# eth-cscs/conflux

Hardware: NVIDIA H100
Metric: LU GFLOP/s (FP64, (2/3)N^3) (higher is better)
Workload: dtype f64

## Files before the change

### conflux_b200/csrc/panel.cu

```cuda
#include <cooperative_groups.h>

#include <climits>
#include <cstdlib>

#include "common.cuh"
#include "kernels.h"

namespace cflx {

namespace {
constexpr int PT_THREADS = 256;
constexpr int PT_WARPS = PT_THREADS / 32;
constexpr int PT_LAUNCH = PT_THREADS + 32;
constexpr int PT_ALLWARPS = PT_LAUNCH / 32;
constexpr int MAXG = 132;
constexpr int RPT_LIMIT = 8;

struct PanelArgs {
    double* W;
    int64_t ldw;
    int n, v, nsteps;
    int R, Rpad, G;
    int* perm_out;
    double* A00;
    uint2* slot_hdr;
    uint2* slot_rows;
    int epoch_base;
};

__device__ __forceinline__ void st_ll(uint2* p, unsigned data, unsigned epoch) {
    asm volatile("st.volatile.global.v2.u32 [%0], {%1, %2};" ::"l"(p), "r"(data), "r"(epoch) : "memory");
}
__device__ __forceinline__ uint4 ld_ll2(const uint2* p) {
    uint4 v;
    asm volatile("ld.volatile.global.v4.u32 {%0, %1, %2, %3}, [%4];" : "=r"(v.x), "=r"(v.y), "=r"(v.z), "=r"(v.w) : "l"(p) : "memory");
    return v;
}

struct Cand {
    unsigned long long key;
    int pos;
    int row;
};

__device__ __forceinline__ Cand warp_argmax(Cand c) {
    const unsigned hi = (unsigned)(c.key >> 32), lo = (unsigned)c.key;
    const unsigned m1 = __reduce_max_sync(0xffffffffu, hi);
    bool in = (hi == m1);
    const unsigned m2 = __reduce_max_sync(0xffffffffu, in ? lo : 0u);
    in = in && (lo == m2);
    const unsigned m3 = __reduce_min_sync(0xffffffffu, in ? (unsigned)c.pos : (unsigned)INT_MAX);
    const unsigned ballot = __ballot_sync(0xffffffffu, in && (unsigned)c.pos == m3);
    const int src = __ffs(ballot) - 1;
    Cand r;
    r.key = ((unsigned long long)m1 << 32) | m2;
    r.pos = (int)m3;
    r.row = __shfl_sync(0xffffffffu, c.row, src);
    return r;
}
__device__ __forceinline__ bool better(const Cand& a, const Cand& b) {
    return a.key > b.key || (a.key == b.key && a.pos < b.pos);
}
__device__ __forceinline__ Cand block_argmax(Cand c, unsigned long long* red_key, int* red_pos, int* red_row, int& rb) {
    Cand w = warp_argmax(c);
    const int warp = threadIdx.x >> 5, lane = threadIdx.x & 31;
    const int o = rb * PT_ALLWARPS;
    rb ^= 1;
    if (lane == 0) {
        red_key[o + warp] = w.key;
        red_pos[o + warp] = w.pos;
        red_row[o + warp] = w.row;
    }
    __syncthreads();
    Cand x{0ull, INT_MAX, -1};
    if (lane < PT_ALLWARPS) x = Cand{red_key[o + lane], red_pos[o + lane], red_row[o + lane]};
    return warp_argmax(x);
}

template <int NB, int RPT_MAX>
__global__ void __launch_bounds__(PT_LAUNCH, 1) panel_getrf_kernel(PanelArgs p) {
    extern __shared__ __align__(16) unsigned char smem_raw[];
    double* Ab = reinterpret_cast<double*>(smem_raw);
    double* U12 = Ab + (size_t)NB * p.Rpad;
    double* LU11 = U12 + (size_t)NB * p.v;
    double* prow = LU11 + NB * (NB + 1);
    unsigned long long* red_key = reinterpret_cast<unsigned long long*>(prow + 2 * (NB + 1));
    int* red_pos = reinterpret_cast<int*>(red_key + 2 * PT_ALLWARPS);
    int* red_row = red_pos + 2 * PT_ALLWARPS;
    int* pivrow_blk = red_row + 2 * PT_ALLWARPS;
    int* win_sh = pivrow_blk + NB;
    unsigned char* s_act = reinterpret_cast<unsigned char*>(win_sh + 4);
    int rb = 0;

    const int t = threadIdx.x, warp = t >> 5, lane = t & 31;
    const bool owner = t < PT_THREADS;
    const bool small = p.G <= 32;
    const bool fetcher = warp == (small ? PT_WARPS : 0);
    const int cta = blockIdx.x;
    const int row_base = cta * p.R;
    const int Rloc = max(0, min(p.R, p.n - row_base));
    const int Rpad = p.Rpad, v = p.v;
    double* __restrict__ W = p.W;
    const int64_t ldw = p.ldw;

    int pos[RPT_MAX];
    bool active[RPT_MAX];
#pragma unroll
    for (int q = 0; q < RPT_MAX; ++q) {
        const int lr = t + q * PT_THREADS;
        pos[q] = row_base + lr;
        active[q] = owner && lr < Rloc;
    }
    for (int lr = t; lr < Rpad; lr += PT_LAUNCH) s_act[lr] = lr < Rloc ? 1 : 0;

    for (int jb = 0; jb < p.nsteps; jb += NB) {
        const int nbc = min(NB, v - jb);
        const int nsb = min(nbc, p.nsteps - jb);
        for (int e = t; e < nbc * Rpad; e += PT_LAUNCH) {
            const int c = e / Rpad, lr = e - c * Rpad;
            if (lr < Rloc) Ab[e] = W[(int64_t)(jb + c) * ldw + row_base + lr];
        }
        __syncthreads();

        auto local_candidate = [&](int col) -> Cand {
            Cand c{0ull, INT_MAX, -1};
#pragma unroll
            for (int q = 0; q < RPT_MAX; ++q) {
                const int lr = t + q * PT_THREADS;
                if (active[q]) {
                    Cand o{(unsigned long long)__double_as_longlong(fabs(Ab[col * Rpad + lr])), pos[q], row_base + lr};
                    if (better(o, c)) c = o;
                }
            }
            return block_argmax(c, red_key, red_pos, red_row, rb);
        };
        auto publish = [&](const Cand& mine, int jg, int jprev, const double* pw) {
            const unsigned epoch = (unsigned)(p.epoch_base + jg + 1);
            const int par = jg & 1;
            uint2* myhdr = p.slot_hdr + (size_t)(par * MAXG + cta) * 4;
            if (t < 4) {
                const unsigned w = t == 0 ? (unsigned)mine.key : t == 1 ? (unsigned)(mine.key >> 32)
                                 : t == 2 ? (unsigned)mine.pos : (unsigned)mine.row;
                st_ll(myhdr + t, w, epoch);
            }
            if (t < nbc) {
                double x = 0.0;
                if (mine.row >= 0) {
                    const int lrw = mine.row - row_base;
                    x = Ab[t * Rpad + lrw];
                    if (jprev >= 0 && t > jprev + 1) x = fma(-Ab[jprev * Rpad + lrw], pw[t], x);
                }
                const unsigned long long xb = (unsigned long long)__double_as_longlong(x);
                uint2* myrow = p.slot_rows + (size_t)(par * MAXG + cta) * 64 + 2 * t;
                st_ll(myrow, (unsigned)xb, epoch);
                st_ll(myrow + 1, (unsigned)(xb >> 32), epoch);
            }
        };
        {
            const Cand mine0 = local_candidate(0);
            if (t < 32) __threadfence();
            publish(mine0, jb, -1, nullptr);
        }
        for (int j = 0; j < nsb; ++j) {
            const int jg = jb + j;
            const int par = jg & 1;
            double* pr = prow + par * (NB + 1);
            if (!small || fetcher) {
                const unsigned epoch = (unsigned)(p.epoch_base + jg + 1);
                Cand gc{0ull, INT_MAX, -1};
                for (int g = small ? lane : t; g < p.G; g += small ? 32 : PT_LAUNCH) {
                    const uint2* h = p.slot_hdr + (size_t)(par * MAXG + g) * 4;
                    uint4 a, b;
                    do {
                        a = ld_ll2(h);
                        b = ld_ll2(h + 2);
                    } while (a.y != epoch || a.w != epoch || b.y != epoch || b.w != epoch);
                    Cand o{((unsigned long long)a.z << 32) | a.x, (int)b.x, (int)b.z};
                    if (better(o, gc)) gc = o;
                }
                const Cand w = small ? warp_argmax(gc) : block_argmax(gc, red_key, red_pos, red_row, rb);
                const int wslot = small ? __ffs(__ballot_sync(0xffffffffu, gc.row == w.row)) - 1 : w.row / p.R;
                if (fetcher && lane < nbc) {
                    const uint2* wr = p.slot_rows + (size_t)(par * MAXG + wslot) * 64 + 2 * lane;
                    uint4 a;
                    do {
                        a = ld_ll2(wr);
                    } while (a.y != epoch || a.w != epoch);
                    const double x = __longlong_as_double((long long)(((unsigned long long)a.z << 32) | a.x));
                    pr[lane] = x;
                    LU11[j * (NB + 1) + lane] = x;
                    if (lane == j) pr[NB] = x != 0.0 ? 1.0 / x : 0.0;
                }
                if (fetcher && lane == 0) {
                    win_sh[2 * par] = w.pos;
                    win_sh[2 * par + 1] = w.row;
                }
            }
            __syncthreads();
            Cand win;
            win.key = 0;
            win.pos = win_sh[2 * par];
            win.row = win_sh[2 * par + 1];
            if (t == 0) {
                pivrow_blk[j] = win.row;
                if (cta == 0) p.perm_out[jg] = win.row;
            }
            const double pivot = pr[j];
            const double rinv = pr[NB];
            const bool have_next = (j + 1 < nbc);
            const double pnext = have_next ? pr[j + 1] : 0.0;
            double lq[RPT_MAX];
#pragma unroll
            for (int q = 0; q < RPT_MAX; ++q) {
                const int lr = t + q * PT_THREADS;
                lq[q] = 0.0;
                if (!active[q]) continue;
                if (row_base + lr == win.row) {
                    active[q] = false;
                    s_act[lr] = 0;
                    continue;
                }
                if (pos[q] == jg) pos[q] = win.pos;
                if (pivot != 0.0) {
                    lq[q] = Ab[j * Rpad + lr] * rinv;
                    Ab[j * Rpad + lr] = lq[q];
                }
                if (have_next) Ab[(j + 1) * Rpad + lr] = fma(-lq[q], pnext, Ab[(j + 1) * Rpad + lr]);
            }
            if (j + 1 < nsb) {
                const Cand mine = local_candidate(j + 1);
                publish(mine, jg + 1, j, pr);
                __syncthreads();
            }
            if (owner) {
                double* __restrict__ ab = Ab;
#pragma unroll 4
                for (int c2 = j + 2; c2 < nbc; ++c2) {
                    const double pc = pr[c2];
#pragma unroll
                    for (int q = 0; q < RPT_MAX; ++q) {
                        const int lr = t + q * PT_THREADS;
                        if (active[q]) ab[c2 * Rpad + lr] = fma(-lq[q], pc, ab[c2 * Rpad + lr]);
                    }
                }
            }
        }

        __syncthreads();
        for (int e = t; e < nbc * Rpad; e += PT_LAUNCH) {
            const int c = e / Rpad, lr = e - c * Rpad;
            if (lr < Rloc) W[(int64_t)(jb + c) * ldw + row_base + lr] = Ab[e];
        }
        if (cta == 0 && p.A00 != nullptr) {
            for (int e = t; e < nsb * nbc; e += PT_LAUNCH) {
                const int i = e / nbc, c = e % nbc;
                p.A00[(size_t)(jb + i) * v + jb + c] = LU11[i * (NB + 1) + c];
            }
        }

        const int cstart = jb + nbc;
        const int rem = v - cstart;
        if (rem > 0) {
            __syncthreads();
            __threadfence();
            for (int cc = t; cc < rem; cc += PT_LAUNCH) {
                const double* col = W + (int64_t)(cstart + cc) * ldw;
                double u[NB];
#pragma unroll
                for (int i = 0; i < NB; ++i) u[i] = (i < nsb) ? ld_cg_f64(col + pivrow_blk[i]) : 0.0;
#pragma unroll
                for (int i = 1; i < NB; ++i) {
                    if (i < nsb) {
#pragma unroll
                        for (int s2 = 0; s2 < i; ++s2) u[i] -= LU11[i * (NB + 1) + s2] * u[s2];
                    }
                }
#pragma unroll
                for (int i = 0; i < NB; ++i) U12[i * v + cc] = u[i];
                if (cta == 0 && p.A00 != nullptr) {
#pragma unroll
                    for (int i = 0; i < NB; ++i)
                        if (i < nsb) p.A00[(size_t)(jb + i) * v + cstart + cc] = u[i];
                }
            }
            __syncthreads();
            auto update_row = [&](int lr, int cfirst, int cstep, bool tail) {
                double l[NB];
#pragma unroll
                for (int i = 0; i < NB; ++i) l[i] = (i < nsb) ? Ab[i * Rpad + lr] : 0.0;
                double* wp = W + (int64_t)cstart * ldw + row_base + lr;
                int cc = cfirst;
                double w0 = 0, w1 = 0, w2 = 0, w3 = 0;
                if (cc + 3 < rem) {
                    w0 = wp[(int64_t)cc * ldw];
                    w1 = wp[(int64_t)(cc + 1) * ldw];
                    w2 = wp[(int64_t)(cc + 2) * ldw];
                    w3 = wp[(int64_t)(cc + 3) * ldw];
                }
                for (; cc + 3 < rem; cc += cstep) {
                    double n0 = 0, n1 = 0, n2 = 0, n3 = 0;
                    const int cn = cc + cstep;
                    if (cn + 3 < rem) {
                        n0 = wp[(int64_t)cn * ldw];
                        n1 = wp[(int64_t)(cn + 1) * ldw];
                        n2 = wp[(int64_t)(cn + 2) * ldw];
                        n3 = wp[(int64_t)(cn + 3) * ldw];
                    }
#pragma unroll
                    for (int i = 0; i < NB; ++i) {
                        const double2 ua = *reinterpret_cast<const double2*>(U12 + i * v + cc);
                        const double2 ub = *reinterpret_cast<const double2*>(U12 + i * v + cc + 2);
                        w0 -= l[i] * ua.x;
                        w1 -= l[i] * ua.y;
                        w2 -= l[i] * ub.x;
                        w3 -= l[i] * ub.y;
                    }
                    wp[(int64_t)cc * ldw] = w0;
                    wp[(int64_t)(cc + 1) * ldw] = w1;
                    wp[(int64_t)(cc + 2) * ldw] = w2;
                    wp[(int64_t)(cc + 3) * ldw] = w3;
                    w0 = n0;
                    w1 = n1;
                    w2 = n2;
                    w3 = n3;
                }
                if (tail) {
                    for (int ct = rem & ~3; ct < rem; ++ct) {
                        double x = wp[(int64_t)ct * ldw];
#pragma unroll
                        for (int i = 0; i < NB; ++i) x -= l[i] * U12[i * v + ct];
                        wp[(int64_t)ct * ldw] = x;
                    }
                }
            };
            if (RPT_MAX == 1 && p.R < PT_THREADS) {
                const int nshare = PT_THREADS / p.R;
                const int lr = t % p.R, part = t / p.R;
                if (owner && part < nshare && lr < Rloc && s_act[lr]) update_row(lr, 4 * part, 4 * nshare, part == 0);
            } else {
#pragma unroll 1
                for (int q = 0; q < RPT_MAX; ++q) {
                    const int lr = t + q * PT_THREADS;
                    if (lr >= Rloc || !active[q]) continue;
                    update_row(lr, 0, 4, true);
                }
            }
        }
        __threadfence();
        __syncthreads();
    }
    if (cta == 0)
        for (int i = p.nsteps + t; i < v; i += PT_LAUNCH) p.perm_out[i] = i;
}

constexpr int SK_CB = 16;
struct StackArgs {
    double* W;
    int64_t ldw;
    int n, v;
    int* perm_out;
    int* ppos;
    unsigned* flags;
    unsigned* ticket;
    unsigned ticket_base, epoch;
};
__device__ __forceinline__ unsigned ld_acquire_u32(const unsigned* p) {
    unsigned v;
    asm volatile("ld.acquire.gpu.global.u32 %0, [%1];" : "=r"(v) : "l"(p) : "memory");
    return v;
}
__device__ __forceinline__ void st_release_u32(unsigned* p, unsigned v) {
    asm volatile("st.release.gpu.global.u32 [%0], %1;" ::"l"(p), "r"(v) : "memory");
}
__device__ __forceinline__ void cp_async16(double* smem_dst, const double* gsrc) {
    asm volatile("cp.async.cg.shared.global [%0], [%1], 16;" ::"r"(smem_u32(smem_dst)), "l"(gsrc) : "memory");
}
__device__ __forceinline__ void cp_async_commit() { asm volatile("cp.async.commit_group;" ::: "memory"); }
__device__ __forceinline__ void cp_async_wait_all() { asm volatile("cp.async.wait_all;" ::: "memory"); }

template <int NT>
__global__ void __launch_bounds__(NT, 1) stack_getrf_kernel(StackArgs p) {
    __shared__ double A12s[SK_CB][SK_CB + 1];
    __shared__ double L11s[SK_CB][SK_CB + 1];
    __shared__ double prow[2][SK_CB];
    __shared__ unsigned long long red_key[2][32];
    __shared__ int red_pos[2][32], red_row[2][32];
    __shared__ int pivs[SK_CB], ppos_s[SK_CB];
    __shared__ int s_cta;
    extern __shared__ __align__(16) double Ls[];
    const int t = threadIdx.x, warp = t >> 5, lane = t & 31, nw = blockDim.x >> 5;
    if (t == 0) s_cta = (int)(atomicAdd(p.ticket, 1u) - p.ticket_base);
    __syncthreads();
    const int c = s_cta, c0 = c * SK_CB;
    const bool valid = t < p.n;
    double* __restrict__ W = p.W;
    const int64_t ldw = p.ldw;
    double a[SK_CB];
#pragma unroll
    for (int j = 0; j < SK_CB; ++j) a[j] = valid ? W[(int64_t)(c0 + j) * ldw + t] : 0.0;
    int pos = t;
    int mypiv = -1;

    for (int b = 0; b < c; ++b) {
        if (t == 0)
            while (ld_acquire_u32(p.flags + b) != p.epoch) {}
        __syncthreads();
        if (t < SK_CB) {
            pivs[t] = ld_cg_s32(p.perm_out + b * SK_CB + t);
            ppos_s[t] = ld_cg_s32(p.ppos + b * SK_CB + t);
        }
        {
            const int half = blockDim.x >> 1, q = t % half, h = t / half;
            if (2 * q < p.n) {
                const double* lp = W + (int64_t)(b * SK_CB + 8 * h) * ldw + 2 * q;
#pragma unroll
                for (int k = 0; k < SK_CB / 2; ++k) cp_async16(Ls + (8 * h + k) * NT + 2 * q, lp + (int64_t)k * ldw);
            }
        }
        cp_async_commit();
        __syncthreads();
        int kk = -1;
        if (mypiv < 0) {
#pragma unroll
            for (int k = 0; k < SK_CB; ++k) {
                if (pivs[k] == t) kk = k;
                else if (kk < 0 && pos == b * SK_CB + k) pos = ppos_s[k];
            }
        }
        if (kk >= 0) {
#pragma unroll
            for (int j = 0; j < SK_CB; ++j) A12s[kk][j] = a[j];
#pragma unroll
            for (int k = 0; k < SK_CB; ++k) L11s[kk][k] = ld_cg_f64(W + (int64_t)(b * SK_CB + k) * ldw + t);
        }
        __syncthreads();
        if (t < SK_CB) {
#pragma unroll
            for (int i = 1; i < SK_CB; ++i) {
                double x = A12s[i][t];
#pragma unroll
                for (int s2 = 0; s2 < i; ++s2) x = fma(-L11s[i][s2], A12s[s2][t], x);
                A12s[i][t] = x;
            }
        }
        cp_async_wait_all();
        __syncthreads();
        if (kk >= 0) {
#pragma unroll
            for (int j = 0; j < SK_CB; ++j) a[j] = A12s[kk][j];
            mypiv = b * SK_CB + kk;
        } else if (mypiv < 0 && valid) {
#pragma unroll
            for (int k = 0; k < SK_CB; ++k) {
                const double lk = Ls[k * NT + t];
#pragma unroll
                for (int j = 0; j < SK_CB; ++j) a[j] = fma(-lk, A12s[k][j], a[j]);
            }
        }
    }

#pragma unroll
    for (int j = 0; j < SK_CB; ++j) {
        const int jg = c0 + j, par = j & 1;
        Cand cd{0ull, INT_MAX, -1};
        if (valid && mypiv < 0) cd = Cand{(unsigned long long)__double_as_longlong(fabs(a[j])), pos, t};
        const Cand w1 = warp_argmax(cd);
        if (lane == 0) {
            red_key[par][warp] = w1.key;
            red_pos[par][warp] = w1.pos;
            red_row[par][warp] = w1.row;
        }
        __syncthreads();
        Cand x{0ull, INT_MAX, -1};
        if (lane < nw) x = Cand{red_key[par][lane], red_pos[par][lane], red_row[par][lane]};
        const Cand win = warp_argmax(x);
        if (t == win.row) {
#pragma unroll
            for (int m = 0; m < SK_CB; ++m) prow[par][m] = a[m];
            mypiv = jg;
        }
        if (t == 0) {
            p.perm_out[jg] = win.row;
            p.ppos[jg] = win.pos;
        }
        __syncthreads();
        if (valid && mypiv < 0) {
            if (pos == jg) pos = win.pos;
            const double pivot = prow[par][j];
            const double rinv = pivot != 0.0 ? 1.0 / pivot : 0.0;
            double lq = 0.0;
            if (pivot != 0.0) {
                lq = a[j] * rinv;
                a[j] = lq;
            }
#pragma unroll
            for (int m = j + 1; m < SK_CB; ++m) a[m] = fma(-lq, prow[par][m], a[m]);
        }
    }
    if (valid) {
#pragma unroll
        for (int j = 0; j < SK_CB; ++j) W[(int64_t)(c0 + j) * ldw + t] = a[j];
    }
    __threadfence();
    __syncthreads();
    if (t == 0) st_release_u32(p.flags + c, p.epoch);
}

int launch_stack_getrf(double* W, int64_t ldw, int n, int v, int* perm_out, PanelWorkspace* ws, cudaStream_t stream) {
    StackArgs a{};
    a.W = W;
    a.ldw = ldw;
    a.n = n;
    a.v = v;
    a.perm_out = perm_out;
    a.ppos = ws->sk_ppos;
    a.flags = ws->sk_flags;
    a.ticket = ws->sk_ticket;
    a.ticket_base = ws->sk_ticket_count;
    a.epoch = ++ws->sk_epoch;
    const int C = v / SK_CB;
    ws->sk_ticket_count += (unsigned)C;
    const int threads = (int)round_up(n, 32);
    static PerDeviceMax cfg;
    if (cfg.raise((size_t)SK_CB * 1024 * sizeof(double))) {
        CFLX_CUDA(cudaFuncSetAttribute(stack_getrf_kernel<1024>, cudaFuncAttributeMaxDynamicSharedMemorySize, SK_CB * 1024 * 8));
        CFLX_CUDA(cudaFuncSetAttribute(stack_getrf_kernel<512>, cudaFuncAttributeMaxDynamicSharedMemorySize, SK_CB * 512 * 8));
    }
    if (threads <= 256) stack_getrf_kernel<256><<<C, threads, SK_CB * 256 * sizeof(double), stream>>>(a);
    else if (threads <= 512) stack_getrf_kernel<512><<<C, threads, SK_CB * 512 * sizeof(double), stream>>>(a);
    else stack_getrf_kernel<1024><<<C, threads, SK_CB * 1024 * sizeof(double), stream>>>(a);
    CFLX_CUDA(cudaGetLastError());
    return CFLX_OK;
}

template <int NB>
size_t panel_smem_bytes(int Rpad, int v) {
    return ((size_t)NB * Rpad + (size_t)NB * v + NB * (NB + 1) + 2 * (NB + 1)) * sizeof(double) +
           2 * PT_ALLWARPS * (sizeof(unsigned long long) + 2 * sizeof(int)) +
           (NB + 4) * sizeof(int) + (size_t)Rpad;
}

int panel_nb(int Rpad, int v) {
    for (int nb = 32; nb >= 4; nb /= 2) {
        const long long limit = 222 * 1024 - (8LL * nb * nb + 796LL * nb + 848);
        if ((nb <= v || nb == 4) && (8LL * nb + 1) * Rpad + 8LL * nb * v <= limit) return nb;
    }
    return 0;
}

template <int NB, int RPT>
int launch_nb_rpt(PanelArgs& a, cudaStream_t stream) {
    const size_t smem = panel_smem_bytes<NB>(a.Rpad, a.v);
    void* params[] = {&a};
    static PerDeviceMax cfg;
    if (cfg.raise(smem))
        CFLX_CUDA(cudaFuncSetAttribute(panel_getrf_kernel<NB, RPT>, cudaFuncAttributeMaxDynamicSharedMemorySize, (int)smem));
    CFLX_CUDA(cudaLaunchCooperativeKernel((void*)panel_getrf_kernel<NB, RPT>, dim3(a.G), dim3(PT_LAUNCH), params, smem, stream));
    return CFLX_OK;
}
template <int NB>
int launch_nb(PanelArgs& a, cudaStream_t stream) {
    const int rpt = (a.R + PT_THREADS - 1) / PT_THREADS;
    if (rpt <= 1) return launch_nb_rpt<NB, 1>(a, stream);
    if (rpt <= 2) return launch_nb_rpt<NB, 2>(a, stream);
    if (rpt <= 4) return launch_nb_rpt<NB, 4>(a, stream);
    return launch_nb_rpt<NB, 8>(a, stream);
}
}


int panel_workspace_create(PanelWorkspace* ws) {
    int dev = 0, sms = 0;
    CFLX_CUDA(cudaGetDevice(&dev));
    CFLX_CUDA(cudaDeviceGetAttribute(&sms, cudaDevAttrMultiProcessorCount, dev));
    ws->max_ctas = sms < MAXG ? sms : MAXG;
    ws->epoch = 1;
    ws->cta_cap = 0;
    CFLX_CUDA(cudaMalloc(&ws->slot_hdr, sizeof(uint2) * 2 * MAXG * 4));
    CFLX_CUDA(cudaMalloc(&ws->slot_rows, sizeof(uint2) * 2 * MAXG * 64));
    CFLX_CUDA(cudaMemset(ws->slot_hdr, 0, sizeof(uint2) * 2 * MAXG * 4));
    CFLX_CUDA(cudaMemset(ws->slot_rows, 0, sizeof(uint2) * 2 * MAXG * 64));
    CFLX_CUDA(cudaMalloc(&ws->sk_flags, sizeof(unsigned) * 1024));
    CFLX_CUDA(cudaMalloc(&ws->sk_ppos, sizeof(int) * 16384));
    CFLX_CUDA(cudaMalloc(&ws->sk_ticket, sizeof(unsigned)));
    CFLX_CUDA(cudaMemset(ws->sk_flags, 0, sizeof(unsigned) * 1024));
    CFLX_CUDA(cudaMemset(ws->sk_ticket, 0, sizeof(unsigned)));
    ws->sk_epoch = 0;
    ws->sk_ticket_count = 0;
    {
        const char* e = getenv("CFLX_STACK_KERNEL");
        ws->sk_enabled = e ? atoi(e) : 1;
    }
    return CFLX_OK;
}
void panel_workspace_destroy(PanelWorkspace* ws) {
    cudaFree(ws->slot_hdr);
    cudaFree(ws->slot_rows);
    cudaFree(ws->sk_flags);
    cudaFree(ws->sk_ppos);
    cudaFree(ws->sk_ticket);
    *ws = PanelWorkspace{};
}

int launch_panel_getrf_a00(double* W, int64_t ldw, int n, int v, int* perm_out, double* A00, int* nb_used,
                           PanelWorkspace* ws, cudaStream_t stream) {
    if (v <= 0 || n < 0) return CFLX_ERR_ARG;
    if (ws->sk_enabled && n >= v && n <= 1024 && v % SK_CB == 0 && v <= 16384 && ldw % 2 == 0 &&
        (reinterpret_cast<uintptr_t>(W) & 15) == 0) {
        if (nb_used) *nb_used = 0;
        return launch_stack_getrf(W, ldw, n, v, perm_out, ws, stream);
    }
    PanelArgs a{};
    a.W = W;
    a.ldw = ldw;
    a.n = n;
    a.v = v;
    a.nsteps = n < v ? n : v;
    int G = (n + 31) / 32;
    if (G < 1) G = 1;
    if (G > ws->max_ctas) G = ws->max_ctas;
    if (ws->cta_cap > 0 && G > ws->cta_cap) {
        G = ws->cta_cap;
        const int need = (n + RPT_LIMIT * PT_THREADS - 1) / (RPT_LIMIT * PT_THREADS);
        if (G < need) G = need < ws->max_ctas ? need : ws->max_ctas;
    }
    int R = (n + G - 1) / G;
    R = (int)round_up(R > 0 ? R : 1, 32);
    G = n > 0 ? (n + R - 1) / R : 1;
    if (R > RPT_LIMIT * PT_THREADS) {
        set_last_error("panel_getrf: n=%d rows exceed the %d-row capacity (%d CTAs x %d rows)", n,
                       ws->max_ctas * RPT_LIMIT * PT_THREADS, ws->max_ctas, RPT_LIMIT * PT_THREADS);
        return CFLX_ERR_UNSUPPORTED;
    }
    a.R = R;
    a.Rpad = R;
    a.G = G;
    a.perm_out = perm_out;
    a.A00 = A00;
    a.slot_hdr = reinterpret_cast<uint2*>(ws->slot_hdr);
    a.slot_rows = reinterpret_cast<uint2*>(ws->slot_rows);
    a.epoch_base = ws->epoch;
    ws->epoch += v + 2 + (v & 1);
    const int nb = panel_nb(a.Rpad, v);
    if (nb == 0) {
        set_last_error("panel_getrf: v=%d with %d rows per CTA exceeds the shared-memory budget of the inner block", v,
                       a.Rpad);
        return CFLX_ERR_UNSUPPORTED;
    }
    if (nb_used) *nb_used = nb;
    switch (nb) {
        case 32: return launch_nb<32>(a, stream);
        case 16: return launch_nb<16>(a, stream);
        case 8: return launch_nb<8>(a, stream);
        default: return launch_nb<4>(a, stream);
    }
}

int launch_panel_getrf(double* W, int64_t ldw, int n, int v, int* perm_out, PanelWorkspace* ws, cudaStream_t stream) {
    return launch_panel_getrf_a00(W, ldw, n, v, perm_out, nullptr, nullptr, ws, stream);
}

}
```

### conflux_b200/csrc/gemm.cu

```cuda
#include <cstdlib>

#include "common.cuh"
#include "kernels.h"

namespace cflx {

namespace {
constexpr int BK = 16, STAGES = 4;

template <int WM, int WN>
struct Cfg {
    static constexpr int BM = 64 * WM, BN = 32 * WN;
    static constexpr int LDA = BM + 4, LDB = BN + 4;
    static constexpr int NCONS = WM * WN, NTHREADS = (NCONS + 1) * 32;
    static constexpr bool STAGE_C = (WM == 2);
    static constexpr int NBAR = 2 * STAGES + (STAGE_C ? WM * STAGES : 0);
    static constexpr size_t SMEM = (size_t)STAGES * BK * (LDA + LDB) * sizeof(double) + NBAR * sizeof(uint64_t);
    static_assert(!STAGE_C || (LDA == LDB && 64 / 16 == STAGES), "one slab per warp row and stage, in both parts");
};

__device__ __forceinline__ double2 ld_c2(const double* p) {
    double2 v;
    asm("ld.global.v2.f64 {%0, %1}, [%2];" : "=d"(v.x), "=d"(v.y) : "l"(p));
    return v;
}

template <int WM, int WN, int MINB>
__global__ void __launch_bounds__(Cfg<WM, WN>::NTHREADS, MINB) gemm_tn_kernel(GemmArgs g) {
    using C = Cfg<WM, WN>;
    constexpr int BM = C::BM, BN = C::BN, LDA = C::LDA, LDB = C::LDB, NCONS = C::NCONS;
    extern __shared__ __align__(128) unsigned char smem_raw[];
    double* sA = reinterpret_cast<double*>(smem_raw);
    double* sB = sA + STAGES * BK * LDA;
    uint64_t* full = reinterpret_cast<uint64_t*>(sB + STAGES * BK * LDB);
    uint64_t* empty = full + STAGES;
    uint64_t* cfull = empty + STAGES;

    const int warp = threadIdx.x >> 5, lane = threadIdx.x & 31;
    const int m0 = blockIdx.y * BM, n0 = blockIdx.x * BN;

    if (threadIdx.x == 0) {
        for (int s = 0; s < STAGES; ++s) {
            mbar_init(&full[s], 1);
            mbar_init(&empty[s], NCONS);
        }
        if constexpr (C::STAGE_C)
            for (int b = 0; b < WM * STAGES; ++b) mbar_init(&cfull[b], 1);
        fence_barrier_init();
    }
    __syncthreads();

    if (warp == NCONS) {
        int wm = g.M - m0;
        wm = wm > BM ? BM : ((wm + 1) & ~1);
        int wn = g.N - n0;
        wn = wn > BN ? BN : ((wn + 1) & ~1);
        const int rr = lane & 15;
        const int nkt = (g.K + BK - 1) / BK;
        const bool use_c = (g.beta != 0.0);
        for (int kt = 0; kt < nkt; ++kt) {
            const int s = kt % STAGES, u = kt / STAGES;
            if (u > 0) mbar_wait(&empty[s], (u - 1) & 1);
            const int rows = min(BK, g.K - kt * BK);
            if (lane == 0) mbar_arrive_expect_tx(&full[s], (uint32_t)(rows * (wm + wn) * sizeof(double)));
            __syncwarp();
            if (rr < rows) {
                const int64_t k = (int64_t)kt * BK + rr;
                if (lane < 16)
                    bulk_g2s(sA + (s * BK + rr) * LDA, g.AT + k * g.ldat + m0, (uint32_t)(wm * sizeof(double)), &full[s]);
                else
                    bulk_g2s(sB + (s * BK + rr) * LDB, g.B + k * g.ldb + n0, (uint32_t)(wn * sizeof(double)), &full[s]);
            }
        }
        if constexpr (C::STAGE_C) {
            if (use_c)
                for (int i = 0; i < STAGES; ++i) {
                    const int s = (nkt + i) % STAGES, kt = nkt + i - STAGES;
                    if (kt >= 0) mbar_wait(&empty[s], (kt / STAGES) & 1);
                    const int wr = lane >> 4, r0 = m0 + 64 * wr + 16 * i;
                    const int rows = max(0, min(16, g.M - r0));
                    uint64_t* bar = &cfull[wr * STAGES + i];
                    if (rr == 0) mbar_arrive_expect_tx(bar, (uint32_t)(rows * wn * sizeof(double)));
                    __syncwarp();
                    if (rr < rows)
                        bulk_g2s(sA + (wr * STAGES + s) * BK * LDA + rr * LDA + 4 * (rr & 1),
                                 g.C + (int64_t)(r0 + rr) * g.ldc + n0, (uint32_t)(wn * sizeof(double)), bar);
                }
        }
        return;
    }

    const int wm_off = (warp / WN) * 64, wn_off = (warp % WN) * 32;
    const int g4 = lane >> 2, t4 = lane & 3;
    double acc[4][4][4];
#pragma unroll
    for (int i = 0; i < 4; ++i)
#pragma unroll
        for (int j = 0; j < 4; ++j) acc[i][j][0] = acc[i][j][1] = acc[i][j][2] = acc[i][j][3] = 0.0;

    int kt = 0;
    for (; kt * BK < g.K; ++kt) {
        const int s = kt % STAGES, u = kt / STAGES;
        mbar_wait(&full[s], u & 1);
        const double* a_s = sA + s * BK * LDA + wm_off + g4;
        const double* b_s = sB + s * BK * LDB + wn_off + g4;
        const int rows = min(BK, g.K - kt * BK);
#pragma unroll
        for (int kk = 0; kk < BK; kk += 8) {
            if (kk < rows) {
                const bool hi = kk + 4 < rows;
                const double* a_k = a_s + (kk + t4) * LDA;
                const double* b_k = b_s + (kk + t4) * LDB;
                double b[4][2];
#pragma unroll
                for (int j = 0; j < 4; ++j) {
                    b[j][0] = b_k[8 * j];
                    b[j][1] = hi ? b_k[4 * LDB + 8 * j] : 0.0;
                }
#pragma unroll
                for (int i = 0; i < 4; ++i) {
                    const double a[4] = {a_k[16 * i], a_k[16 * i + 8], hi ? a_k[4 * LDA + 16 * i] : 0.0,
                                         hi ? a_k[4 * LDA + 16 * i + 8] : 0.0};
#pragma unroll
                    for (int j = 0; j < 4; ++j) dmma16x8x8(acc[i][j], a, b[j]);
                }
            }
        }
        __syncwarp();
        if (lane == 0) mbar_arrive(&empty[s]);
    }

    const double alpha = g.alpha, beta = g.beta;
    const bool use_c = (beta != 0.0);
    const int row0 = m0 + wm_off + g4, col0 = n0 + wn_off + 2 * t4;
    if constexpr (C::STAGE_C) {
        const int wr = warp / WN, nkt = kt;
#pragma unroll
        for (int i = 0; i < 4; ++i) {
            const double* cs = sA + (wr * STAGES + (nkt + i) % STAGES) * BK * LDA + 4 * (g4 & 1) + wn_off + 2 * t4;
            if (use_c) mbar_wait(&cfull[wr * STAGES + i], 0);
#pragma unroll
            for (int h = 0; h < 2; ++h) {
                const int row = row0 + 16 * i + 8 * h;
#pragma unroll
                for (int j = 0; j < 4; ++j) {
                    const int col = col0 + 8 * j;
                    if (row < g.M && col < g.N) {
                        double2 cv = make_double2(0.0, 0.0);
                        if (use_c) cv = *reinterpret_cast<const double2*>(cs + (g4 + 8 * h) * LDA + 8 * j);
                        double2 out;
                        out.x = fma(alpha, acc[i][j][2 * h], beta * cv.x);
                        out.y = fma(alpha, acc[i][j][2 * h + 1], beta * cv.y);
                        *reinterpret_cast<double2*>(g.D + (int64_t)row * g.ldd + col) = out;
                    }
                }
            }
        }
    } else {
#pragma unroll
        for (int sl = 0; sl < 8; ++sl) {
            const int row = row0 + 8 * sl;
            double2 cv[4];
#pragma unroll
            for (int j = 0; j < 4; ++j) {
                const int col = col0 + 8 * j;
                cv[j] = make_double2(0.0, 0.0);
                if (use_c && row < g.M && col < g.N) cv[j] = ld_c2(g.C + (int64_t)row * g.ldc + col);
            }
#pragma unroll
            for (int j = 0; j < 4; ++j) {
                const int col = col0 + 8 * j;
                if (row < g.M && col < g.N) {
                    double2 out;
                    out.x = fma(alpha, acc[sl / 2][j][2 * (sl & 1)], beta * cv[j].x);
                    out.y = fma(alpha, acc[sl / 2][j][2 * (sl & 1) + 1], beta * cv[j].y);
                    *reinterpret_cast<double2*>(g.D + (int64_t)row * g.ldd + col) = out;
                }
            }
        }
    }
}
}

namespace {
template <int WM, int WN, int MINB>
int setup_one() {
    static PerDeviceMax cfg;
    if (cfg.raise(Cfg<WM, WN>::SMEM))
        CFLX_CUDA(cudaFuncSetAttribute(gemm_tn_kernel<WM, WN, MINB>, cudaFuncAttributeMaxDynamicSharedMemorySize,
                                       (int)Cfg<WM, WN>::SMEM));
    return CFLX_OK;
}
template <int WM, int WN, int MINB>
int launch_one(const GemmArgs& g, cudaStream_t stream) {
    using C = Cfg<WM, WN>;
    CFLX_TRY((setup_one<WM, WN, MINB>()));
    dim3 grid((g.N + C::BN - 1) / C::BN, (g.M + C::BM - 1) / C::BM);
    gemm_tn_kernel<WM, WN, MINB><<<grid, C::NTHREADS, C::SMEM, stream>>>(g);
    CFLX_CUDA(cudaGetLastError());
    return CFLX_OK;
}
int tile_variant() {
    static int v = -1;
    if (v < 0) {
        const char* e = getenv("CFLX_GEMM_TILE");
        v = (e && atoi(e) == 64) ? 64 : 128;
    }
    return v;
}
}

int gemm_tn_setup() {
    CFLX_TRY((setup_one<2, 4, 1>()));
    CFLX_TRY((setup_one<1, 4, 2>()));
    return CFLX_OK;
}

int launch_gemm_tn(const GemmArgs& g, cudaStream_t stream) {
    if (g.M <= 0 || g.N <= 0 || g.K <= 0) return CFLX_OK;
    if ((g.K & 3) || (g.N & 1) || (g.ldat & 1) || (g.ldb & 1) || (g.ldc & 1) || (g.ldd & 1)) {
        set_last_error("gemm_tn: unsupported shape M=%d N=%d K=%d ld=(%lld,%lld,%lld,%lld)", g.M, g.N, g.K,
                       (long long)g.ldat, (long long)g.ldb, (long long)g.ldc, (long long)g.ldd);
        return CFLX_ERR_UNSUPPORTED;
    }
    if (tile_variant() == 64) return launch_one<1, 4, 2>(g, stream);
    return launch_one<2, 4, 1>(g, stream);
}

}
```

Before: 25220.

## Keep next panel block in shared memory, pad layouts, fast-path warp argmax

The trailing update now writes the first NB columns of the next inner block straight into shared memory, so the block no longer has to be reloaded from global memory at each step. Only the first block is loaded explicitly, and rows that are already eliminated are filled from global. Rpad is now R+1 and the U12 leading dimension is padded to even, which changes the shared-memory layout and is meant to reduce bank conflicts. The warp argmax also returns early when one lane holds a unique top key, skipping the extra reductions. This adds complexity around row activity and layout, and the extra padding raises shared-memory use, which can change which NB gets chosen.

```diff
diff --git a/conflux_b200/csrc/panel.cu b/conflux_b200/csrc/panel.cu
--- a/conflux_b200/csrc/panel.cu
+++ b/conflux_b200/csrc/panel.cu
@@ -47,6 +47,15 @@
     const unsigned hi = (unsigned)(c.key >> 32), lo = (unsigned)c.key;
     const unsigned m1 = __reduce_max_sync(0xffffffffu, hi);
     bool in = (hi == m1);
+    const unsigned top = __ballot_sync(0xffffffffu, in);
+    if ((top & (top - 1)) == 0) {
+        const int src = __ffs(top) - 1;
+        Cand r;
+        r.key = ((unsigned long long)m1 << 32) | __shfl_sync(0xffffffffu, lo, src);
+        r.pos = __shfl_sync(0xffffffffu, c.pos, src);
+        r.row = __shfl_sync(0xffffffffu, c.row, src);
+        return r;
+    }
     const unsigned m2 = __reduce_max_sync(0xffffffffu, in ? lo : 0u);
     in = in && (lo == m2);
     const unsigned m3 = __reduce_min_sync(0xffffffffu, in ? (unsigned)c.pos : (unsigned)INT_MAX);
@@ -81,8 +90,9 @@
 __global__ void __launch_bounds__(PT_LAUNCH, 1) panel_getrf_kernel(PanelArgs p) {
     extern __shared__ __align__(16) unsigned char smem_raw[];
     double* Ab = reinterpret_cast<double*>(smem_raw);
+    const int ldu = p.v + (p.v & 1);
     double* U12 = Ab + (size_t)NB * p.Rpad;
-    double* LU11 = U12 + (size_t)NB * p.v;
+    double* LU11 = U12 + (size_t)NB * ldu;
     double* prow = LU11 + NB * (NB + 1);
     unsigned long long* red_key = reinterpret_cast<unsigned long long*>(prow + 2 * (NB + 1));
     int* red_pos = reinterpret_cast<int*>(red_key + 2 * PT_ALLWARPS);
@@ -116,11 +126,14 @@
     for (int jb = 0; jb < p.nsteps; jb += NB) {
         const int nbc = min(NB, v - jb);
         const int nsb = min(nbc, p.nsteps - jb);
-        for (int e = t; e < nbc * Rpad; e += PT_LAUNCH) {
-            const int c = e / Rpad, lr = e - c * Rpad;
-            if (lr < Rloc) Ab[e] = W[(int64_t)(jb + c) * ldw + row_base + lr];
-        }
-        __syncthreads();
+        if (jb == 0) {
+            for (int c = 0, lr = t;; lr += PT_LAUNCH) {
+                for (; lr >= Rpad; lr -= Rpad) ++c;
+                if (c >= nbc) break;
+                if (lr < Rloc) Ab[c * Rpad + lr] = W[(int64_t)(jb + c) * ldw + row_base + lr];
+            }
+            __syncthreads();
+        }
 
         auto local_candidate = [&](int col) -> Cand {
             Cand c{0ull, INT_MAX, -1};
@@ -247,10 +260,8 @@
         }
 
         __syncthreads();
-        for (int e = t; e < nbc * Rpad; e += PT_LAUNCH) {
-            const int c = e / Rpad, lr = e - c * Rpad;
-            if (lr < Rloc) W[(int64_t)(jb + c) * ldw + row_base + lr] = Ab[e];
-        }
+        for (int c = 0; c < nbc; ++c)
+            for (int lr = t; lr < Rloc; lr += PT_LAUNCH) W[(int64_t)(jb + c) * ldw + row_base + lr] = Ab[c * Rpad + lr];
         if (cta == 0 && p.A00 != nullptr) {
             for (int e = t; e < nsb * nbc; e += PT_LAUNCH) {
                 const int i = e / nbc, c = e % nbc;
@@ -276,19 +287,30 @@
                     }
                 }
 #pragma unroll
-                for (int i = 0; i < NB; ++i) U12[i * v + cc] = u[i];
+                for (int i = 0; i < NB; ++i) U12[i * ldu + cc] = u[i];
                 if (cta == 0 && p.A00 != nullptr) {
 #pragma unroll
                     for (int i = 0; i < NB; ++i)
                         if (i < nsb) p.A00[(size_t)(jb + i) * v + cstart + cc] = u[i];
                 }
             }
+            const int nbn = min(NB, rem);
+            auto load_l = [&](int lr, double (&l)[NB]) {
+#pragma unroll
+                for (int i = 0; i < NB; ++i) l[i] = (i < nsb) ? Ab[i * Rpad + lr] : 0.0;
+            };
+            const bool shared_rows = RPT_MAX == 1 && p.R < PT_THREADS;
+            const int lr_sh = t % p.R, part = t / p.R, nshare = PT_THREADS / p.R;
+            const bool mine = shared_rows && owner && part < nshare && lr_sh < Rloc && s_act[lr_sh];
+            for (int lr = t; lr < Rloc; lr += PT_LAUNCH)
+                if (!s_act[lr])
+                    for (int c = 0; c < nbn; ++c) Ab[c * Rpad + lr] = W[(int64_t)(cstart + c) * ldw + row_base + lr];
+            double l_sh[NB];
+            if (mine) load_l(lr_sh, l_sh);
             __syncthreads();
-            auto update_row = [&](int lr, int cfirst, int cstep, bool tail) {
-                double l[NB];
-#pragma unroll
-                for (int i = 0; i < NB; ++i) l[i] = (i < nsb) ? Ab[i * Rpad + lr] : 0.0;
+            auto update_row = [&](int lr, const double (&l)[NB], int cfirst, int cstep, bool tail) {
                 double* wp = W + (int64_t)cstart * ldw + row_base + lr;
+                double* ap = Ab + lr;
                 int cc = cfirst;
                 double w0 = 0, w1 = 0, w2 = 0, w3 = 0;
                 if (cc + 3 < rem) {
@@ -308,17 +330,24 @@
                     }
 #pragma unroll
                     for (int i = 0; i < NB; ++i) {
-                        const double2 ua = *reinterpret_cast<const double2*>(U12 + i * v + cc);
-                        const double2 ub = *reinterpret_cast<const double2*>(U12 + i * v + cc + 2);
+                        const double2 ua = *reinterpret_cast<const double2*>(U12 + i * ldu + cc);
+                        const double2 ub = *reinterpret_cast<const double2*>(U12 + i * ldu + cc + 2);
                         w0 -= l[i] * ua.x;
                         w1 -= l[i] * ua.y;
                         w2 -= l[i] * ub.x;
                         w3 -= l[i] * ub.y;
                     }
-                    wp[(int64_t)cc * ldw] = w0;
-                    wp[(int64_t)(cc + 1) * ldw] = w1;
-                    wp[(int64_t)(cc + 2) * ldw] = w2;
-                    wp[(int64_t)(cc + 3) * ldw] = w3;
+                    if (cc < nbn) {
+                        ap[cc * Rpad] = w0;
+                        ap[(cc + 1) * Rpad] = w1;
+                        ap[(cc + 2) * Rpad] = w2;
+                        ap[(cc + 3) * Rpad] = w3;
+                    } else {
+                        wp[(int64_t)cc * ldw] = w0;
+                        wp[(int64_t)(cc + 1) * ldw] = w1;
+                        wp[(int64_t)(cc + 2) * ldw] = w2;
+                        wp[(int64_t)(cc + 3) * ldw] = w3;
+                    }
                     w0 = n0;
                     w1 = n1;
                     w2 = n2;
@@ -328,21 +357,22 @@
                     for (int ct = rem & ~3; ct < rem; ++ct) {
                         double x = wp[(int64_t)ct * ldw];
 #pragma unroll
-                        for (int i = 0; i < NB; ++i) x -= l[i] * U12[i * v + ct];
-                        wp[(int64_t)ct * ldw] = x;
+                        for (int i = 0; i < NB; ++i) x -= l[i] * U12[i * ldu + ct];
+                        if (ct < nbn) ap[ct * Rpad] = x;
+                        else wp[(int64_t)ct * ldw] = x;
                     }
                 }
             };
-            if (RPT_MAX == 1 && p.R < PT_THREADS) {
-                const int nshare = PT_THREADS / p.R;
-                const int lr = t % p.R, part = t / p.R;
-                if (owner && part < nshare && lr < Rloc && s_act[lr]) update_row(lr, 4 * part, 4 * nshare, part == 0);
+            if (shared_rows) {
+                if (mine) update_row(lr_sh, l_sh, 4 * part, 4 * nshare, part == 0);
             } else {
 #pragma unroll 1
                 for (int q = 0; q < RPT_MAX; ++q) {
                     const int lr = t + q * PT_THREADS;
                     if (lr >= Rloc || !active[q]) continue;
-                    update_row(lr, 0, 4, true);
+                    double l[NB];
+                    load_l(lr, l);
+                    update_row(lr, l, 0, 4, true);
                 }
             }
         }
@@ -535,15 +565,15 @@
 
 template <int NB>
 size_t panel_smem_bytes(int Rpad, int v) {
-    return ((size_t)NB * Rpad + (size_t)NB * v + NB * (NB + 1) + 2 * (NB + 1)) * sizeof(double) +
+    return ((size_t)NB * Rpad + (size_t)NB * (v + (v & 1)) + NB * (NB + 1) + 2 * (NB + 1)) * sizeof(double) +
            2 * PT_ALLWARPS * (sizeof(unsigned long long) + 2 * sizeof(int)) +
            (NB + 4) * sizeof(int) + (size_t)Rpad;
 }
 
-int panel_nb(int Rpad, int v) {
+int panel_nb(int R, int v) {
     for (int nb = 32; nb >= 4; nb /= 2) {
         const long long limit = 222 * 1024 - (8LL * nb * nb + 796LL * nb + 848);
-        if ((nb <= v || nb == 4) && (8LL * nb + 1) * Rpad + 8LL * nb * v <= limit) return nb;
+        if ((nb <= v || nb == 4) && (8LL * nb + 1) * R + 8LL * nb * v <= limit) return nb;
     }
     return 0;
 }
@@ -633,7 +663,7 @@
         return CFLX_ERR_UNSUPPORTED;
     }
     a.R = R;
-    a.Rpad = R;
+    a.Rpad = R + 1;
     a.G = G;
     a.perm_out = perm_out;
     a.A00 = A00;
@@ -641,10 +671,10 @@
     a.slot_rows = reinterpret_cast<uint2*>(ws->slot_rows);
     a.epoch_base = ws->epoch;
     ws->epoch += v + 2 + (v & 1);
-    const int nb = panel_nb(a.Rpad, v);
+    const int nb = panel_nb(a.R, v);
     if (nb == 0) {
         set_last_error("panel_getrf: v=%d with %d rows per CTA exceeds the shared-memory budget of the inner block", v,
-                       a.Rpad);
+                       a.R);
         return CFLX_ERR_UNSUPPORTED;
     }
     if (nb_used) *nb_used = nb;
```

Measured after the change: 25700, median of 6. 1.02x the previous value.

## Group GEMM tiles for L2 reuse and stream C/D with evict-first hints

Applied to the files above, without the earlier changes.

Replaces the 2D grid with a 1D grid that visits tiles in column-major groups of 1024 rows, so consecutive blocks share A and B panels in L2. C loads (bulk copies) and D stores in the staged-C path now carry an L2 evict_first policy, so streaming output does not push reused operands out of L2. This adds per-block index arithmetic and depends on the hint behaving as intended on the trailing update's access pattern.

```diff
diff --git a/conflux_b200/csrc/gemm.cu b/conflux_b200/csrc/gemm.cu
--- a/conflux_b200/csrc/gemm.cu
+++ b/conflux_b200/csrc/gemm.cu
@@ -7,10 +7,13 @@
 
 namespace {
 constexpr int BK = 16, STAGES = 4;
+
+constexpr int GROUP_ROWS = 1024;
 
 template <int WM, int WN>
 struct Cfg {
     static constexpr int BM = 64 * WM, BN = 32 * WN;
+    static constexpr int GM = GROUP_ROWS / BM;
     static constexpr int LDA = BM + 4, LDB = BN + 4;
     static constexpr int NCONS = WM * WN, NTHREADS = (NCONS + 1) * 32;
     static constexpr bool STAGE_C = (WM == 2);
@@ -23,6 +26,31 @@
     double2 v;
     asm("ld.global.v2.f64 {%0, %1}, [%2];" : "=d"(v.x), "=d"(v.y) : "l"(p));
     return v;
+}
+
+__device__ __forceinline__ uint64_t l2_evict_first() {
+    uint64_t pol;
+    asm("createpolicy.fractional.L2::evict_first.b64 %0, 1.0;" : "=l"(pol));
+    return pol;
+}
+__device__ __forceinline__ void bulk_g2s_evict_first(void* smem_dst, const void* gsrc, uint32_t bytes, uint64_t* bar,
+                                                     uint64_t pol) {
+    asm volatile("cp.async.bulk.shared::cluster.global.mbarrier::complete_tx::bytes.L2::cache_hint [%0], [%1], %2, [%3], %4;"
+                 ::"r"(smem_u32(smem_dst)), "l"(gsrc), "r"(bytes), "r"(smem_u32(bar)), "l"(pol)
+                 : "memory");
+}
+__device__ __forceinline__ void st_d2_evict_first(double* p, double2 v, uint64_t pol) {
+    asm volatile("st.global.L2::cache_hint.v2.f64 [%0], {%1, %2}, %3;" ::"l"(p), "d"(v.x), "d"(v.y), "l"(pol));
+}
+
+template <int WM, int WN>
+__device__ __forceinline__ void tile_origin(const GemmArgs& g, int& m0, int& n0) {
+    using C = Cfg<WM, WN>;
+    const int mtiles = (g.M + C::BM - 1) / C::BM, ntiles = (g.N + C::BN - 1) / C::BN;
+    const int grp = blockIdx.x / (C::GM * ntiles), r = blockIdx.x - grp * C::GM * ntiles;
+    const int gsz = min(C::GM, mtiles - grp * C::GM);
+    m0 = (grp * C::GM + r % gsz) * C::BM;
+    n0 = (r / gsz) * C::BN;
 }
 
 template <int WM, int WN, int MINB>
@@ -37,7 +65,6 @@
     uint64_t* cfull = empty + STAGES;
 
     const int warp = threadIdx.x >> 5, lane = threadIdx.x & 31;
-    const int m0 = blockIdx.y * BM, n0 = blockIdx.x * BN;
 
     if (threadIdx.x == 0) {
         for (int s = 0; s < STAGES; ++s) {
@@ -51,6 +78,8 @@
     __syncthreads();
 
     if (warp == NCONS) {
+        int m0, n0;
+        tile_origin<WM, WN>(g, m0, n0);
         int wm = g.M - m0;
         wm = wm > BM ? BM : ((wm + 1) & ~1);
         int wn = g.N - n0;
@@ -83,8 +112,9 @@
                     if (rr == 0) mbar_arrive_expect_tx(bar, (uint32_t)(rows * wn * sizeof(double)));
                     __syncwarp();
                     if (rr < rows)
-                        bulk_g2s(sA + (wr * STAGES + s) * BK * LDA + rr * LDA + 4 * (rr & 1),
-                                 g.C + (int64_t)(r0 + rr) * g.ldc + n0, (uint32_t)(wn * sizeof(double)), bar);
+                        bulk_g2s_evict_first(sA + (wr * STAGES + s) * BK * LDA + rr * LDA + 4 * (rr & 1),
+                                             g.C + (int64_t)(r0 + rr) * g.ldc + n0, (uint32_t)(wn * sizeof(double)),
+                                             bar, l2_evict_first());
                 }
         }
         return;
@@ -132,6 +162,8 @@
 
     const double alpha = g.alpha, beta = g.beta;
     const bool use_c = (beta != 0.0);
+    int m0, n0;
+    tile_origin<WM, WN>(g, m0, n0);
     const int row0 = m0 + wm_off + g4, col0 = n0 + wn_off + 2 * t4;
     if constexpr (C::STAGE_C) {
         const int wr = warp / WN, nkt = kt;
@@ -151,7 +183,7 @@
                         double2 out;
                         out.x = fma(alpha, acc[i][j][2 * h], beta * cv.x);
                         out.y = fma(alpha, acc[i][j][2 * h + 1], beta * cv.y);
-                        *reinterpret_cast<double2*>(g.D + (int64_t)row * g.ldd + col) = out;
+                        st_d2_evict_first(g.D + (int64_t)row * g.ldd + col, out, l2_evict_first());
                     }
                 }
             }
@@ -195,7 +227,7 @@
 int launch_one(const GemmArgs& g, cudaStream_t stream) {
     using C = Cfg<WM, WN>;
     CFLX_TRY((setup_one<WM, WN, MINB>()));
-    dim3 grid((g.N + C::BN - 1) / C::BN, (g.M + C::BM - 1) / C::BM);
+    const int grid = ((g.N + C::BN - 1) / C::BN) * ((g.M + C::BM - 1) / C::BM);
     gemm_tn_kernel<WM, WN, MINB><<<grid, C::NTHREADS, C::SMEM, stream>>>(g);
     CFLX_CUDA(cudaGetLastError());
     return CFLX_OK;
```

Measured after the change: 25270 before, 25880 after, median of 6. +2.4%, better.
